# interestingLSY/swiftLLM

Measured on AMD Instinct MI355X. Metric: decode tok/s (llama3-8b bfloat16, batch 32/GPU, 1024-in/128-out; prefill tok/s alongside), higher is better.
Workload: dtype bf16

## Files before the change

include/swiftllm_hip.h:

```cpp
#ifndef SWIFTLLM_HIP_H
#define SWIFTLLM_HIP_H

#include <stddef.h>
#include <stdint.h>

#ifdef __cplusplus
extern "C" {
#endif

#define SWL_ABI_VERSION 2

#define SWL_F16 0
#define SWL_BF16 1

#define SWL_OK 0
#define SWL_ERR_BAD_ARG (-1)
#define SWL_ERR_UNSUPPORTED (-2)
#define SWL_ERR_LAUNCH (-3)
#define SWL_ERR_RUNTIME (-4)

typedef void *swl_stream_t;

int swl_abi_version(void);
const char *swl_strerror(int code);
// ... 215 lines not shown
int swl_gemm_packed_wide_silu_gate(void *out, const void *x, const void *w_up_gate_packed, int32_t M, int32_t I,
                                   int32_t K, int64_t x_row_stride, int64_t out_row_stride, int32_t waves_per_group,
                                   int32_t dtype, swl_stream_t stream);
int swl_gemm_packed_mid_partial(float *slabs, size_t slabs_bytes, const void *x, const void *w_packed, int32_t M,
                                int32_t N, int32_t K, int64_t x_row_stride, int32_t k_splits, int32_t dtype,
                                swl_stream_t stream);

int swl_gemm_skinny_choose_splits(int32_t N, int32_t K);
int swl_gemm_skinny_packed_choose_splits(int32_t N, int32_t K);
int swl_gemm_skinny_partial(float *slabs, size_t slabs_bytes, const void *x, const void *w, int32_t M,
                            int32_t N, int32_t K, int64_t x_row_stride, int32_t k_splits,
                            int32_t dtype, swl_stream_t stream);
int swl_splitk_reduce(void *out, const float *slabs, int32_t k_splits, int32_t M, int32_t N,
                      int64_t out_row_stride, int32_t dtype, swl_stream_t stream);
int swl_splitk_fused_add_rmsnorm(void *x_out, void *residual, const void *w, float eps,
                                 const float *slabs, int32_t k_splits, int64_t num_tokens,
                                 int32_t hidden, int32_t dtype, swl_stream_t stream);
int swl_splitk_rotary_store_kv_decode(void *q_out, void *k_out, void *v_out, const float *qkv_slabs,
                                      int32_t k_splits, const void *cos_table, const void *sin_table,
                                      const int32_t *pos_idx, void *k_cache, void *v_cache,
                                      const int32_t *block_table, const int32_t *seq_ids,
                                      const int32_t *seq_lens, int32_t num_decoding_seqs,
                                      int32_t num_q_heads, int32_t num_kv_heads, int32_t head_dim,
                                      int32_t cur_layer, int32_t num_layers, int32_t block_size,
                                      int32_t max_blocks_per_seq, int64_t q_tok_stride,
                                      int64_t k_tok_stride, int64_t v_tok_stride, int32_t dtype,
                                      swl_stream_t stream);

int swl_decode_positions(int32_t *pos_idx, const int32_t *seq_lens, int32_t num_decoding_seqs,
                         swl_stream_t stream);

int swl_splitk_add_scale(void *x_scaled, void *residual, const void *w, const float *slabs, int32_t k_splits,
                         float *ssq_out, int64_t num_tokens, int32_t hidden, int32_t dtype, swl_stream_t stream);
int swl_gemm_skinny_packed_silu_gate_rs(void *out, const void *x, const void *w_up_gate_packed, const float *row_ssq,
                                        int32_t ssq_parts, float eps, int32_t M, int32_t I, int32_t K,
                                        int64_t x_row_stride, int64_t out_row_stride, int32_t dtype, swl_stream_t stream);
int swl_paged_attn_decode_qkv_rs(void *o, const float *qkv_slabs, int32_t k_splits, const float *row_ssq,
                                 int32_t ssq_parts, int32_t hidden, float eps, const void *cos_table,
                                 const void *sin_table, const int32_t *pos_idx, void *k_cache, void *v_cache,
                                 const int32_t *block_table, const int32_t *seq_ids, const int32_t *seq_lens,
                                 void *scratch, float softmax_scale, int32_t num_decoding_seqs, int32_t num_q_heads,
                                 int32_t num_kv_heads, int32_t head_dim, int32_t num_layers, int32_t block_size,
                                 int32_t cur_layer, int32_t max_blocks_per_seq, int32_t seq_block_size,
                                 int32_t num_seq_blocks, int64_t o_tok_stride, int32_t dtype, swl_stream_t stream);

int swl_paged_attn_decode_qkv_rs_partials(void *o, const float *qkv_slabs, int32_t k_splits, const float *row_ssq,
                                          int32_t ssq_parts, int32_t hidden, float eps, const void *cos_table,
                                          const void *sin_table, const int32_t *pos_idx, void *k_cache, void *v_cache,
                                          const int32_t *block_table, const int32_t *seq_ids, const int32_t *seq_lens,
                                          void *scratch, float softmax_scale, int32_t num_decoding_seqs,
                                          int32_t num_q_heads, int32_t num_kv_heads, int32_t head_dim,
                                          int32_t num_layers, int32_t block_size, int32_t cur_layer,
                                          int32_t max_blocks_per_seq, int32_t seq_block_size, int32_t num_seq_blocks,
                                          int64_t o_tok_stride, int32_t dtype, swl_stream_t stream);
int swl_gemm_tiny_partial_from_attn(float *slabs_out, size_t slabs_out_bytes, int32_t k_splits_out,
                                    const float *attn_scratch, const int32_t *seq_lens, int32_t num_q_heads,
                                    int32_t head_dim, int32_t seq_block_size, int32_t num_seq_blocks,
                                    const void *w_packed, int32_t M, int32_t N, int32_t dtype, swl_stream_t stream);
int swl_gemm_tiny_max_tokens(void);
int swl_gemm_tiny_partial_from_splitk(float *slabs_out, size_t slabs_out_bytes, int32_t k_splits_out, float *ssq_out,
                                      const float *slabs_in, int32_t k_splits_in, const void *residual_in,
                                      void *residual_out, const void *norm_w, const void *w_packed, int32_t M, int32_t N,
                                      int32_t K, int32_t dtype, swl_stream_t stream);
int swl_gemm_tiny_silu_gate_from_splitk(void *out, const float *slabs_in, int32_t k_splits_in, const void *residual_in,
                                        void *residual_out, const void *norm_w, float eps, const void *w_up_gate_packed,
                                        int32_t M, int32_t I, int32_t K, int64_t out_row_stride, int32_t dtype,
// ... 49 lines not shown
```

swiftllm_amd/_hip.py:

```python
import ctypes
import os
import threading

import torch

_LIB_NAME = "libswiftllm_hip.so"
_LIB_PATH = os.path.join(os.path.dirname(os.path.abspath(__file__)), "csrc", _LIB_NAME)

SWL_F16 = 0
SWL_BF16 = 1
ABI_VERSION = 2

_P = ctypes.c_void_p
_I32 = ctypes.c_int32
_I64 = ctypes.c_int64
_F32 = ctypes.c_float

SIGNATURES = {
    "swl_rmsnorm": [_P, _P, _F32, _I64, _I32, _I32, _P],
    "swl_fused_add_rmsnorm": [_P, _P, _P, _F32, _I64, _I32, _I32, _P],
    "swl_rotary": [_P, _P, _P, _P, _P, _I64, _I32, _I32, _I32, _I64, _I64, _I32, _P],
    "swl_store_kv_prefill": [_P, _P, _P, _P, _P, _P, _P, _P, _I32, _I32, _I32, _I32, _I32, _I32,
                             _I32, _I32, _I64, _I64, _I32, _P],
    "swl_store_kv_decode": [_P, _P, _P, _P, _P, _P, _P, _I32, _I32, _I32, _I32, _I32, _I32, _I32,
# ... 49 lines not shown
    "swl_gemm_skinny_partial": [_P, ctypes.c_size_t, _P, _P, _I32, _I32, _I32, _I64, _I32, _I32, _P],
    "swl_splitk_reduce": [_P, _P, _I32, _I32, _I32, _I64, _I32, _P],
    "swl_gemm_skinny_silu_gate": [_P, _P, _P, _I32, _I32, _I32, _I64, _I64, _I32, _P],
    "swl_splitk_fused_add_rmsnorm": [_P, _P, _P, _F32, _P, _I32, _I64, _I32, _I32, _P],
    "swl_splitk_add_scale": [_P, _P, _P, _P, _I32, _P, _I64, _I32, _I32, _P],
    "swl_gemm_skinny_packed_silu_gate_rs": [_P, _P, _P, _P, _I32, _F32, _I32, _I32, _I32, _I64, _I64, _I32, _P],
    "swl_paged_attn_decode_qkv_rs": [_P, _P, _I32, _P, _I32, _I32, _F32, _P, _P, _P, _P, _P, _P, _P, _P, _P, _F32, _I32,
                                     _I32, _I32, _I32, _I32, _I32, _I32, _I32, _I32, _I32, _I64, _I32, _P],
    "swl_splitk_rotary_store_kv_decode": [_P, _P, _P, _P, _I32, _P, _P, _P, _P, _P, _P, _P, _P, _I32, _I32,
                                          _I32, _I32, _I32, _I32, _I32, _I32, _I64, _I64, _I64, _I32, _P],
    "swl_paged_attn_decode_qkv_rs_partials": [_P, _P, _I32, _P, _I32, _I32, _F32, _P, _P, _P, _P, _P, _P, _P, _P, _P, _F32,
                                              _I32, _I32, _I32, _I32, _I32, _I32, _I32, _I32, _I32, _I32, _I64, _I32, _P],
    "swl_gemm_tiny_partial_from_attn": [_P, ctypes.c_size_t, _I32, _P, _P, _I32, _I32, _I32, _I32, _P, _I32, _I32, _I32, _P],
    "swl_gemm_tiny_partial_from_splitk": [_P, ctypes.c_size_t, _I32, _P, _P, _I32, _P, _P, _P, _P, _I32, _I32, _I32, _I32, _P],
    "swl_gemm_tiny_silu_gate_from_splitk": [_P, _P, _I32, _P, _P, _P, _F32, _P, _I32, _I32, _I32, _I64, _I32, _P],
    "swl_gemm_rows_add": [_P, _P, _P, _I32, _I32, _I32, _I64, _I32, _P],
    "swl_gemm_skinny_packed_partial_nf": [_P, ctypes.c_size_t, _P, _P, _P, _P, _I32, _I32, _I32, _I64, _I32, _I32, _P],
    "swl_gemm_skinny_packed_silu_gate_nf": [_P, _P, _P, _F32, _P, _I32, _I32, _I32, _I64, _I64, _I32, _P],
    "swl_gemm_rows_add_ssq": [_P, _P, _P, _P, _I32, _I32, _I32, _I64, _I32, _P],
    "swl_gemm_skinny_packed_silu_gate_nx": [_P, _P, _P, _F32, _P, _I32, _P, _I32, _I32, _I32, _I64, _I64, _I32, _P],
    "swl_gemm_skinny_packed_partial_nx": [_P, ctypes.c_size_t, _P, _P, _F32, _P, _I32, _P, _I32, _I32, _I32, _I64, _I32, _I32, _P],
    "swl_decode_engine_reset": [_P, ctypes.c_size_t, _P],
    "swl_decode_engine_step": [_P, _P, _P, _P, _P, _P, _P, _P, _P, _P, _P, _P, _P, ctypes.c_size_t, _P, _P, _I32, _I32,
                               _I32, _I32, _I32, _I32, _I32, _F32, _F32, _I32, _I32, _P],
}
_SPECIAL = {
    "swl_abi_version": ([], _I32),
    "swl_strerror": ([_I32], ctypes.c_char_p),
    "swl_paged_attn_scratch_bytes": ([_I32, _I32, _I32, _I32], ctypes.c_size_t),
    "swl_argmax_scratch_bytes": ([_I64], ctypes.c_size_t),
    "swl_gemm_skinny_workspace_bytes": ([_I32, _I32, _I32], ctypes.c_size_t),
    "swl_gemm_skinny_choose_splits": ([_I32, _I32], _I32),
    "swl_gemm_skinny_packed_choose_splits": ([_I32, _I32], _I32),
    "swl_gemm_packed_mid_choose_splits": ([_I32, _I32, _I32], _I32),
    "swl_gemm_packed_wide_workspace_bytes": ([_I32, _I32, _I32], ctypes.c_size_t),
    "swl_gemm_packed_wide_choose_splits": ([_I32, _I32, _I32], _I32),
    "swl_gemm_tiny_max_tokens": ([], _I32),
    "swl_gemm_rows_supported": ([_I32, _I32, _I32], _I32),
    "swl_decode_engine_supported": ([_I32, _I32, _I32, _I32, _I32, _I32], _I32),
    "swl_decode_engine_slots_per_layer": ([_I32, _I32, _I32, _I32], _I32),
    "swl_decode_engine_workspace_bytes": ([_I32, _I32, _I32, _I32], ctypes.c_size_t),
    "swl_paged_attn_verify_max_tokens": ([_I32, _I32], _I32),
    "swl_paged_attn_verify": ([_P, _P, _P, _P, _P, _P, _P, _P, _P, _P, _F32, _I32, _I32, _I32, _I32, _I32, _I32, _I32,
                               _I32, _I32, _I32, _I32, _I32, _I32, _I64, _I64, _I32, _P], _I32),
    "swl_logits_adjust": ([_P, _I64, _I32, _I64, _I32, _P, _P, _P, _P, _P, _P], _I32),
    "swl_lora_k_splits": ([_I32], _I32),
    "swl_lora_shrink": ([_P, _P, _P, _P, _P, _I32, _I32, _I32, _I32, _I32, _I64, _I32, _P], _I32),
    "swl_lora_expand": ([_P, _P, _P, _P, _P, _P, _P, _I32, _I32, _I32, _I32, _I32, _I32, _I32, _I32, _I64, _I32, _P], _I32),
}

_lock = threading.Lock()
_lib = None


class HipLibraryError(RuntimeError):
    """libswiftllm_hip.so is missing, stale, or a kernel entry point returned an error code."""


def library_path() -> str:
    return os.environ.get("SWIFTLLM_HIP_LIB", _LIB_PATH)


def load():
    global _lib
    if _lib is not None:
        return _lib
# ... 71 lines not shown
```

swiftllm_amd/csrc/build.py:

```python
import argparse
import concurrent.futures
import os
import shutil
import subprocess
import tempfile

HERE = os.path.dirname(os.path.abspath(__file__))
ROOT = os.path.dirname(os.path.dirname(HERE))
SOURCES = [
    "rmsnorm.hip",
    "rotary.hip",
    "kvcache.hip",
    "silu_mul.hip",
    "paged_attn.hip",
    "paged_attn_verify.hip",
    "prefill_attn.hip",
    "prefill_attn_paged.hip",
    "kvcache_fp8.hip",
    "paged_attn_fp8.hip",
    "block_table.hip",
    "swap_blocks.hip",
    "gemm_skinny.hip",
    "gemm_tiny.hip",
    "gemm_wide.hip",
    "gemm_rows.hip",
    "argmax.hip",
    "sampling.hip",
    "logits_adjust.hip",
    "lora.hip",
    "decode_engine.hip",
]
HEADERS = ["swl_common.h", "attend_block.h", "attn_mfma.h", "decode_attn.h", "prefill_tile.h", "fp8_kv.h", "gemm_host.h", os.path.join(ROOT, "include", "swiftllm_hip.h")]
LIB = os.path.join(HERE, "libswiftllm_hip.so")
OBJ_DIR = os.path.join(HERE, "build")
ARCH = "gfx950"
CXXFLAGS = [f"--offload-arch={ARCH}", "-O3", "-std=c++17", "-fPIC", "-ffp-contract=off", "-Wall",
            "-Wno-unused-function"]


def _hipcc() -> str:
    for cand in (os.environ.get("HIPCC"), shutil.which("hipcc"), "/opt/rocm/bin/hipcc"):
        if cand and os.path.exists(cand):
            return cand
    raise RuntimeError("hipcc not found (set HIPCC or install ROCm under /opt/rocm)")


def _newer(target: str, deps) -> bool:
    if not os.path.exists(target):
        return False
    t = os.path.getmtime(target)
    return all(os.path.getmtime(d) <= t for d in deps)


def build(force: bool = False, jobs: int = 0, verbose: bool = True, tag: str = "", defines=(), swap=None) -> str:
    hipcc = _hipcc()
    obj_dir = os.path.join(tempfile.gettempdir(), "swiftllm_hip_variants", tag) if tag else OBJ_DIR
    lib = os.path.join(HERE, f"libswiftllm_hip_{tag}.so") if tag else LIB
    return _build(hipcc, obj_dir, lib, [f"-D{d}" for d in defines], force, jobs, verbose, swap or {})


def _build(hipcc, OBJ_DIR, LIB, extra, force, jobs, verbose, swap) -> str:
    os.makedirs(OBJ_DIR, exist_ok=True)
    hdrs = [h if os.path.isabs(h) else os.path.join(HERE, h) for h in HEADERS]
    hdrs.append(os.path.abspath(__file__))
    todo, objs = [], []
# ... 41 lines not shown
```

swiftllm_amd/csrc/gemm_skinny.hip:

```cpp
#include "gemm_host.h"

namespace swl {

__device__ __forceinline__ float16_t mfma32x32x16(vec8_t<f16> a, vec8_t<f16> b, float16_t c) {
    return __builtin_amdgcn_mfma_f32_32x32x16_f16(a, b, c, 0, 0, 0);
}
__device__ __forceinline__ float16_t mfma32x32x16(vec8_t<bf16> a, vec8_t<bf16> b, float16_t c) {
    return __builtin_amdgcn_mfma_f32_32x32x16_bf16(a, b, c, 0, 0, 0);
}

constexpr int kKT = 128;
constexpr int kGemmWaves = 4;

enum GemmMode {
    kGemmDirect = 0,
    kGemmPartial = 1,
    kGemmSiluGate = 2,
};

struct GemmExtra {
    int k_tiles_total;
    const float *ssq_in;
    float eps;
    int ssq_parts;
    const void *norm_w;
    float *ssq_out;
};

template <typename T, int MODE>
__device__ __forceinline__ void gemm_epilogue(const float16_t &acc, void *__restrict__ out_, T *wtiles,
                                              int wave_pitch, int wave, int lane, bool is_gate, bool tile_ok,
                                              int col0, int n0, int ksplit, int M, int N, int64_t out_stride,
                                              float rs = 1.0f, int gate_waves_off = 2) {
    const int l32 = lane & 31;
    const int hf = lane >> 5;
    if constexpr (MODE == kGemmSiluGate) {
        T *mine = wtiles + wave * wave_pitch;
        if (is_gate) {
#pragma unroll
            for (int r = 0; r < 16; ++r) {
                const float g = to_f(to_t<T>(acc[r] * rs));
                mine[l32 * 40 + (r & 3) + 8 * (r >> 2) + 4 * hf] = to_t<T>(g / (1.0f + expf(-g)));
            }
        }
        __syncthreads();
// ... 337 lines not shown
        }
        gemm_epilogue<T, MODE>(acc, out_, &lds[0][0], 32 * 40, wave, lane, is_gate, tile_ok, col0, n0, ksplit, M, N,
                               out_stride, rs, HWV);
    } else {
        gemm_epilogue<T, MODE>(acc, out_, &lds[PACKED ? 0 : 2][0], 32 * kKT, wave, lane, is_gate, tile_ok, col0, n0,
                               ksplit, M, N, out_stride);
    }
}

template <typename T>
__global__ __launch_bounds__(256) void splitk_reduce_kernel(T *__restrict__ out,
                                                            const float *__restrict__ slabs, int M,
                                                            int N, int KS, int64_t out_stride) {
    const int n4 = N >> 2;
    const int64_t items = static_cast<int64_t>(M) * n4;
    for (int64_t it = blockIdx.x * 256ll + threadIdx.x; it < items;
         it += static_cast<int64_t>(gridDim.x) * 256ll) {
        const int m = static_cast<int>(it / n4);
        const int c = static_cast<int>(it - static_cast<int64_t>(m) * n4);
        float4_t s = {0.f, 0.f, 0.f, 0.f};
        for (int k = 0; k < KS; ++k) {
            const float4_t v = *reinterpret_cast<const float4_t *>(
                slabs + (static_cast<int64_t>(k) * M + m) * N + 4 * c);
            s += v;
        }
        typedef T vec4 __attribute__((ext_vector_type(4)));
        vec4 o;
#pragma unroll
        for (int e = 0; e < 4; ++e) o[e] = to_t<T>(s[e]);
        *reinterpret_cast<vec4 *>(out + static_cast<int64_t>(m) * out_stride + 4 * c) = o;
    }
}

static int choose_k_splits(int N, int K) {
    const int tiles = N / 32;
    int ks = 1;
    while (ks < 16 && tiles * ks < 768 && K % (kKT * ks * 2) == 0 && K / (ks * 2) >= 2 * kKT) ks *= 2;
    return ks;
}

static int choose_k_splits_packed(int N, int K, bool *uneven) {
    const int even = choose_k_splits(N, K);
    *uneven = false;
    const int tiles = N / 32, ktiles = K / kKT;
    if (tiles * even >= 512) return even;
    int ks = even;
    while (ks < 16 && tiles * ks < 768 && ktiles / (ks * 2) >= 8) ks *= 2;
    if (ks == even) return even;
    *uneven = K % (kKT * ks) != 0;
    return ks;
}

static bool use_ring(int kc) { return kc / kKT >= 8; }

template <typename T>
void launch_splitk_reduce(T *out, const float *slabs, int ks, int M, int N, int64_t out_row_stride, hipStream_t stream) {
    const int64_t items = static_cast<int64_t>(M) * (N / 4);
    hipLaunchKernelGGL((splitk_reduce_kernel<T>), dim3(static_cast<unsigned>((items + 255) / 256)), dim3(256), 0, stream,
                       out, slabs, M, N, ks, out_row_stride);
}
template void launch_splitk_reduce<f16>(f16 *, const float *, int, int, int, int64_t, hipStream_t);
template void launch_splitk_reduce<bf16>(bf16 *, const float *, int, int, int, int64_t, hipStream_t);

template <int MODE>
static int four_wave_groups(int N) {
    return MODE == kGemmSiluGate ? (N / 32 + 1) / 2 : (N / 32 + kGemmWaves - 1) / kGemmWaves;
}

static GemmArgs silu_gate_args(void *out, const void *x, const void *w, int M, int I, int K, int64_t x_row_stride,
                               int64_t out_row_stride, int max_m = 32) {
    return GemmArgs{out, x, w, nullptr, 0, M, I, K, x_row_stride, out_row_stride, 1, max_m, kKT};
}

template <typename T, int MODE>
static void launch_rowmajor(const GemmArgs &a, hipStream_t stream, void *dst, int64_t dst_stride, int kc, int ks) {
    const dim3 grid(four_wave_groups<MODE>(a.N), ks);
    const T *x = static_cast<const T *>(a.x), *w = static_cast<const T *>(a.w);
    if (use_ring(kc))
        hipLaunchKernelGGL((gemm_skinny_ring_kernel<T, MODE>), grid, dim3(kGemmWaves * 64), 0, stream, dst, x, w, a.M, a.N,
                           a.K, kc, a.x_row_stride, dst_stride, GemmExtra{});
    else
        hipLaunchKernelGGL((gemm_skinny_kernel<T, MODE>), grid, dim3(kGemmWaves * 64), 0, stream, dst, x, w, a.M, a.N, a.K,
                           kc, a.x_row_stride, dst_stride);
}

template <typename T>
static int run_gemm(const GemmArgs &a, hipStream_t stream) {
    const int ks = a.k_splits > 0 ? a.k_splits : choose_k_splits(a.N, a.K);
    if (a.K % (kKT * ks) != 0) return SWL_ERR_UNSUPPORTED;
    const int kc = a.K / ks;
    return run_splitk<T>(
        a, ks, stream,
        [&](void *out) { launch_rowmajor<T, kGemmDirect>(a, stream, out, a.out_row_stride, kc, ks); },
        [&](float *slabs) { launch_rowmajor<T, kGemmPartial>(a, stream, slabs, a.N, kc, ks); });
}

}

extern "C" size_t swl_gemm_skinny_workspace_bytes(int32_t M, int32_t N, int32_t K) {
// ... 40 lines not shown
    if (!out || !slabs || out_row_stride < N || (out_row_stride & 3)) return SWL_ERR_BAD_ARG;
    if (!swl::aligned16(slabs) || (reinterpret_cast<uintptr_t>(out) & 7u)) return SWL_ERR_BAD_ARG;
    SWL_DISPATCH_DTYPE(dtype, T, {
        swl::launch_splitk_reduce<T>(static_cast<T *>(out), slabs, k_splits, M, N, out_row_stride,
                                     static_cast<hipStream_t>(stream));
    });
    return swl::check_launch();
}

extern "C" int swl_gemm_skinny_silu_gate(void *out, const void *x, const void *w_up_gate, int32_t M,
                                         int32_t I, int32_t K, int64_t x_row_stride,
                                         int64_t out_row_stride, int32_t dtype, swl_stream_t stream) {
    const swl::GemmArgs a = swl::silu_gate_args(out, x, w_up_gate, M, I, K, x_row_stride, out_row_stride);
    int rc;
    if (swl::gemm_args_settled(a, rc)) return rc;
    SWL_DISPATCH_DTYPE(dtype, T, {
        swl::launch_rowmajor<T, swl::kGemmSiluGate>(a, static_cast<hipStream_t>(stream), out, out_row_stride, K, 1);
    });
    return swl::check_launch();
}

namespace swl {

template <typename T>
__global__ __launch_bounds__(256) void pack_weight_kernel(T *__restrict__ dst, const T *__restrict__ src, int N, int K) {
    const int64_t blocks = static_cast<int64_t>(N / 32) * (K / 16);
    const int lane = threadIdx.x & 63;
    for (int64_t b = blockIdx.x * 4ll + (threadIdx.x >> 6); b < blocks; b += gridDim.x * 4ll) {
        const int64_t nt = b / (K / 16);
        const int k16 = static_cast<int>(b - nt * (K / 16));
        const T *s = src + (nt * 32 + (lane & 31)) * K + k16 * 16 + 8 * (lane >> 5);
        store8(dst + (b * 64 + lane) * 8, load8(s));
    }
}

static bool prefer_three_waves(int N, int ks) {
    const int tiles = N / 32;
    if (tiles % 3 != 0) return false;
    const int wg4 = (tiles + kGemmWaves - 1) / kGemmWaves * ks, wg3 = tiles / 3 * ks;
    return wg4 < 256 && wg3 <= 256;
}

static bool silu_gate_two_waves(int M) {
    static const int forced = [] { const char *e = getenv("SWL_SILU_WAVES"); return !e ? 0 : e[0] == '2' ? 2 : e[0] == '4' ? 4 : 0; }();
    return forced ? forced == 2 : M <= 8;
}

template <typename T, int MODE, bool NF = false, bool NX = false>
static void launch_packed_ring(const GemmArgs &a, hipStream_t stream, void *dst, int64_t dst_stride, int kc, int ks,
                               const GemmExtra &fuse = GemmExtra{}) {
    const int tiles = a.N / 32;
    auto launch = [&](auto rd, auto nwv, int groups) {
        constexpr int RD = decltype(rd)::value, NWV = decltype(nwv)::value;
        hipLaunchKernelGGL((gemm_skinny_ring_kernel<T, MODE, true, RD, NWV, NF, NX>), dim3(groups, ks), dim3(NWV * 64), 0,
                           stream, dst, static_cast<const T *>(a.x), static_cast<const T *>(a.w), a.M, a.N, a.K, kc,
                           a.x_row_stride, dst_stride, fuse);
    };
    const bool deep = use_ring(kc);
    if constexpr (MODE == kGemmPartial) {
        if (fuse.k_tiles_total == 0 && prefer_three_waves(a.N, ks)) {
            if (NF || !deep) return launch(IntTag<2>{}, IntTag<3>{}, tiles / 3);
            if constexpr (!NF) return launch(IntTag<3>{}, IntTag<3>{}, tiles / 3);
        }
    }
    if constexpr (MODE == kGemmSiluGate && NF) {
        if (deep && (NX ? a.M <= 8 : silu_gate_two_waves(a.M))) return launch(IntTag<3>{}, IntTag<2>{}, tiles);
    }
    const int groups = four_wave_groups<MODE>(a.N);
    if (deep) return launch(IntTag<3>{}, IntTag<kGemmWaves>{}, groups);
    if constexpr (!(MODE == kGemmSiluGate && NX)) launch(IntTag<2>{}, IntTag<kGemmWaves>{}, groups);
}

template <typename T>
static int run_gemm_packed(const GemmArgs &a, hipStream_t stream) {
    bool uneven = false;
    int ks = a.k_splits;
    if (ks <= 0) ks = choose_k_splits_packed(a.N, a.K, &uneven);
    else uneven = a.K % (kKT * ks) != 0;
    if (uneven && (a.K / kKT) / ks < 8) return SWL_ERR_UNSUPPORTED;
    const int kc = uneven ? (a.K / kKT / ks) * kKT : a.K / ks;
    GemmExtra fuse{};
    fuse.k_tiles_total = uneven ? a.K / kKT : 0;
    return run_splitk<T>(
        a, ks, stream, [&](void *out) { launch_packed_ring<T, kGemmDirect>(a, stream, out, a.out_row_stride, kc, ks); },
        [&](float *slabs) { launch_packed_ring<T, kGemmPartial>(a, stream, slabs, a.N, kc, ks, fuse); });
}

}

extern "C" int swl_gemm_pack_weight(void *dst, const void *src, int32_t N, int32_t K, int32_t dtype,
                                    swl_stream_t stream) {
    if (N <= 0 || K <= 0 || !dst || !src || dst == src) return SWL_ERR_BAD_ARG;
    if ((N & 31) || (K & 15)) return SWL_ERR_UNSUPPORTED;
    if (!swl::aligned16(dst) || !swl::aligned16(src)) return SWL_ERR_BAD_ARG;
    const int64_t blocks = static_cast<int64_t>(N / 32) * (K / 16);
    const unsigned grid = static_cast<unsigned>(blocks / 4 + 1 < 65536 ? blocks / 4 + 1 : 65536);
    SWL_DISPATCH_DTYPE(dtype, T, {
        hipLaunchKernelGGL((swl::pack_weight_kernel<T>), dim3(grid), dim3(256), 0, static_cast<hipStream_t>(stream),
                           static_cast<T *>(dst), static_cast<const T *>(src), N, K);
    });
    return swl::check_launch();
}

extern "C" int swl_gemm_skinny_packed(void *out, const void *x, const void *w_packed, void *workspace,
                                      size_t workspace_bytes, int32_t M, int32_t N, int32_t K, int64_t x_row_stride,
                                      int64_t out_row_stride, int32_t k_splits, int32_t dtype, swl_stream_t stream) {
    const swl::GemmArgs a{out, x, w_packed, workspace, workspace_bytes, M, N, K, x_row_stride, out_row_stride, k_splits, 32,
                          swl::kKT};
    int rc;
    if (swl::gemm_args_settled(a, rc)) return rc;
    SWL_DISPATCH_DTYPE(dtype, T, { return swl::run_gemm_packed<T>(a, static_cast<hipStream_t>(stream)); });
}

extern "C" int swl_gemm_skinny_packed_partial(float *slabs, size_t slabs_bytes, const void *x, const void *w_packed,
                                              int32_t M, int32_t N, int32_t K, int64_t x_row_stride,
// ... 370 lines not shown
```

swiftllm_amd/csrc/rmsnorm.hip:

```cpp
#include "swl_common.h"

namespace swl {

template <int NWAVES>
__device__ __forceinline__ float block_allreduce_sum(float v, float *lds) {
    v = wave_allreduce_sum(v);
    if constexpr (NWAVES > 1) {
        const int wave = threadIdx.x >> 6;
        if ((threadIdx.x & 63) == 0) lds[wave] = v;
        __syncthreads();
        float t = 0.f;
#pragma unroll
        for (int i = 0; i < NWAVES; ++i) t += lds[i];
        v = t;
    }
    return v;
}

template <typename T, int NT, int VPT, bool FUSED_ADD>
__global__ __launch_bounds__(NT) void rmsnorm_kernel(T *__restrict__ x, T *__restrict__ residual,
                                                     const T *__restrict__ w, float eps, int hidden,
                                                     const float *__restrict__ slabs, int ks,
                                                     int64_t slab_stride) {
    __shared__ float red[NT / 64];
    const int64_t row = blockIdx.x;
    const int nvec = hidden >> 3;
    T *xr = x + row * hidden;
    T *rr = FUSED_ADD ? residual + row * hidden : nullptr;

    vec8_t<T> wv[VPT];
#pragma unroll
    for (int i = 0; i < VPT; ++i) {
        const int v = threadIdx.x + i * NT;
// ... 11 lines not shown
                vec8_t<T> rv = load8(rr + v * 8);
#pragma unroll
                for (int j = 0; j < 8; ++j) xv[j] = add_t<T>(xv[j], rv[j]);
                store8(rr + v * 8, xv);
            }
#pragma unroll
            for (int j = 0; j < 8; ++j) {
                vals[i][j] = to_f(xv[j]);
                ssq = fmaf(vals[i][j], vals[i][j], ssq);
            }
        } else {
#pragma unroll
            for (int j = 0; j < 8; ++j) vals[i][j] = 0.f;
        }
    }
    ssq = block_allreduce_sum<NT / 64>(ssq, red);
    const float variance = ssq / static_cast<float>(hidden);
    const float rstd = 1.0f / sqrtf(variance + eps);
#pragma unroll
    for (int i = 0; i < VPT; ++i) {
        const int v = threadIdx.x + i * NT;
        if (v < nvec) {
            vec8_t<T> ov;
#pragma unroll
            for (int j = 0; j < 8; ++j) ov[j] = to_t<T>(vals[i][j] * rstd * to_f(wv[i][j]));
            store8(xr + v * 8, ov);
        }
    }
}

constexpr int kAddScaleThreads = 128;
constexpr int kAddScaleChunk = kAddScaleThreads * 8;

template <typename T>
__global__ __launch_bounds__(kAddScaleThreads) void splitk_add_scale_kernel(
    T *__restrict__ xs, T *__restrict__ residual, const T *__restrict__ w, const float *__restrict__ slabs, int ks,
    int64_t slab_stride, float *__restrict__ ssq_out, int num_tokens, int hidden) {
    __shared__ float red[kAddScaleThreads / 64];
    const int part = blockIdx.x, row = blockIdx.y;
    const int col = part * kAddScaleChunk + threadIdx.x * 8;
    const int64_t off = static_cast<int64_t>(row) * hidden + col;
    const vec8_t<T> wv = load8(w + col);
    const vec8_t<T> rv = load8(residual + off);
    vec8_t<T> xv = load8_splitk<T>(slabs, ks, slab_stride, off);
    vec8_t<T> sv;
    float ssq = 0.f;
#pragma unroll
    for (int j = 0; j < 8; ++j) {
        xv[j] = add_t<T>(xv[j], rv[j]);
        const float v = to_f(xv[j]);
        ssq = fmaf(v, v, ssq);
        sv[j] = to_t<T>(v * to_f(wv[j]));
    }
    store8(residual + off, xv);
    store8(xs + off, sv);
    ssq = block_allreduce_sum<kAddScaleThreads / 64>(ssq, red);
    if (threadIdx.x == 0) ssq_out[static_cast<int64_t>(part) * num_tokens + row] = ssq;
}

template <typename T, bool FUSED_ADD>
static int launch_rmsnorm(T *x, T *residual, const T *w, float eps, int64_t num_tokens, int hidden,
                          hipStream_t stream, const float *slabs = nullptr, int ks = 0) {
    const int64_t slab_stride = num_tokens * hidden;
    const int nvec = hidden / 8;
    const dim3 grid(static_cast<unsigned>(num_tokens));
#define SWL_RMS_CASE(NT, VPT)                                                                    \
    hipLaunchKernelGGL((rmsnorm_kernel<T, NT, VPT, FUSED_ADD>), grid, dim3(NT), 0, stream, x,    \
                       residual, w, eps, hidden, slabs, ks, slab_stride)
    if (nvec <= 64) SWL_RMS_CASE(64, 1);
    else if (nvec <= 128) SWL_RMS_CASE(128, 1);
    else if (nvec <= 256) SWL_RMS_CASE(256, 1);
// ... 33 lines not shown
        return swl::launch_rmsnorm<T, true>(static_cast<T *>(x), static_cast<T *>(residual),
                                            static_cast<const T *>(w), eps, num_tokens, hidden,
                                            static_cast<hipStream_t>(stream));
    });
}

extern "C" int swl_splitk_fused_add_rmsnorm(void *x_out, void *residual, const void *w, float eps,
                                            const float *slabs, int32_t k_splits,
                                            int64_t num_tokens, int32_t hidden, int32_t dtype,
                                            swl_stream_t stream) {
    if (num_tokens < 0 || hidden <= 0 || (hidden & 7) || k_splits <= 0) return SWL_ERR_BAD_ARG;
    if (num_tokens == 0) return SWL_OK;
    if (!x_out || !residual || !w || !slabs || !swl::aligned16(x_out) || !swl::aligned16(residual) ||
        !swl::aligned16(w) || !swl::aligned16(slabs))
        return SWL_ERR_BAD_ARG;
    if (num_tokens > 0x7fffffffLL) return SWL_ERR_UNSUPPORTED;
    SWL_DISPATCH_DTYPE(dtype, T, {
        return swl::launch_rmsnorm<T, true>(static_cast<T *>(x_out), static_cast<T *>(residual),
                                            static_cast<const T *>(w), eps, num_tokens, hidden,
                                            static_cast<hipStream_t>(stream), slabs, k_splits);
    });
}

extern "C" int swl_splitk_add_scale(void *x_scaled, void *residual, const void *w, const float *slabs, int32_t k_splits,
                                    float *ssq_out, int64_t num_tokens, int32_t hidden, int32_t dtype,
                                    swl_stream_t stream) {
    if (num_tokens < 0 || hidden <= 0 || k_splits <= 0) return SWL_ERR_BAD_ARG;
    if (num_tokens == 0) return SWL_OK;
    if (hidden % swl::kAddScaleChunk) return SWL_ERR_UNSUPPORTED;
    if (!x_scaled || !residual || !w || !slabs || !ssq_out || !swl::aligned16(x_scaled) || !swl::aligned16(residual) ||
        !swl::aligned16(w) || !swl::aligned16(slabs))
        return SWL_ERR_BAD_ARG;
    if (num_tokens > 65535) return SWL_ERR_UNSUPPORTED;
    const dim3 grid(hidden / swl::kAddScaleChunk, static_cast<unsigned>(num_tokens));
    SWL_DISPATCH_DTYPE(dtype, T, {
        hipLaunchKernelGGL((swl::splitk_add_scale_kernel<T>), grid, dim3(swl::kAddScaleThreads), 0,
                           static_cast<hipStream_t>(stream), static_cast<T *>(x_scaled), static_cast<T *>(residual),
                           static_cast<const T *>(w), slabs, k_splits, num_tokens * static_cast<int64_t>(hidden), ssq_out,
                           static_cast<int>(num_tokens), hidden);
    });
    return swl::check_launch();
}
```

swiftllm_amd/engine_config.py:

```python
import argparse
import dataclasses


@dataclasses.dataclass
class EngineConfig:
    model_path: str
    use_dummy: bool

    block_size: int
    gpu_mem_utilization: float
    num_cpu_blocks: int
    max_seqs_in_block_table: int
    max_blocks_per_seq: int

    max_batch_size: int
    max_tokens_in_batch: int

    dtype: str = "float16"
    fuse_qkv: bool = True
    use_hip_graph: bool = True
    use_skinny_gemm: bool = True
    pack_decode_weights: bool = True
    tuning: dict = None
    max_prefill_chunk: int = 0
    kv_cache_dtype: str = "auto"
    speculative_ngram: int = 0
    speculative_max_batch: int = 8
    max_loras: int = 0
    max_lora_rank: int = 16
    lora_modules: list = None

    TUNING_DEFAULTS = dict(
        fuse_rope_kvstore=True,
        fuse_splitk_consumers=True,
        fuse_rope_into_attention=True,
        defer_rmsnorm=True,
        tiny_decode_batches=True,
        rows_decode=True,
        decode_engine=False,
        pin_swap_memory=True,
        pause_gc_while_serving=True,
    )

    SUPPORTED_BLOCK_SIZE = 16
    KV_CACHE_DTYPES = ("auto", "fp8_e4m3")
    LORA_RANKS = (8, 16, 32, 64)

    def __post_init__(self):
        if int(self.block_size) != self.SUPPORTED_BLOCK_SIZE:
            raise ValueError(
                f"block_size={self.block_size} is not supported: the MI355X kernels are built for "
                f"{self.SUPPORTED_BLOCK_SIZE}-token KV blocks (pass --block-size {self.SUPPORTED_BLOCK_SIZE})")
        if self.dtype not in ("float16", "bfloat16"):
            raise ValueError(f"dtype must be 'float16' or 'bfloat16', got {self.dtype!r}")
        if int(self.max_prefill_chunk) < 0:
            raise ValueError(f"max_prefill_chunk must be >= 0 (0 = off), got {self.max_prefill_chunk}")
        if self.kv_cache_dtype not in self.KV_CACHE_DTYPES:
            raise ValueError(f"kv_cache_dtype must be one of {list(self.KV_CACHE_DTYPES)}, got {self.kv_cache_dtype!r}")
        if int(self.speculative_ngram) < 0:
            raise ValueError(f"speculative_ngram must be >= 0 (0 = off), got {self.speculative_ngram}")
        if int(self.speculative_max_batch) < 0:
            raise ValueError(f"speculative_max_batch must be >= 0, got {self.speculative_max_batch}")
        if int(self.max_loras) < 0:
            raise ValueError(f"max_loras must be >= 0 (0 = off), got {self.max_loras}")
        if int(self.max_lora_rank) not in self.LORA_RANKS:
            raise ValueError(f"max_lora_rank must be one of {list(self.LORA_RANKS)}, got {self.max_lora_rank}")
        if self.lora_modules:
            if int(self.max_loras) <= 0:
                raise ValueError("lora_modules needs max_loras > 0")
            names = [str(m).partition("=")[0] for m in self.lora_modules]
            if any("=" not in str(m) or not n or not str(m).partition("=")[2] for m, n in zip(self.lora_modules, names)):
                raise ValueError(f"lora_modules entries are 'NAME=PATH' strings, got {list(self.lora_modules)}")
# ... 66 lines not shown
```

swiftllm_amd/worker/model.py:

```python
import math
import os
import time
from typing import List, Optional

import torch

from swiftllm_amd import _hip
from swiftllm_amd.engine_config import EngineConfig
from swiftllm_amd.model_config import LlamaModelConfig
from swiftllm_amd.sampling_params import SamplingParams, is_greedy
from swiftllm_amd.utils import GB

from .batch_plan import BatchPlan, plan_batch, plan_verify
from .block_manager import BlockManager
from . import decode_engine as _decode_engine
from .infer_state import LlamaInferState
from .kernels.block_swapping import swap_blocks
from .kernels.linear import RawResidual
from .kernels.paged_attn import verify_max_tokens
from .kernels.rmsnorm import fused_add_rmsnorm_from_splitk, rmsnorm_inplace
from .kernels import logits_process
from .kernels.sampling import device_args, pack_params
from .lora import LoraBatch, LoraStaging, LoraStep, LoraStore, parse_lora_modules, rows_of_sequences
from .layers.pre_layer import LlamaPreLayer
from .layers.transformer_layer import LlamaTransformerLayer
from .layers.post_layer import LlamaPostLayer
from .token_history import TokenHistory, row_entries
from .weight import load_weights, pack_decode_weights

_DTYPES = {"float16": torch.float16, "fp16": torch.float16, "half": torch.float16,
           "bfloat16": torch.bfloat16, "bf16": torch.bfloat16}


def _require_hip_device():
    if not torch.cuda.is_available():
        raise _hip.HipLibraryError(
            "no HIP device visible: swiftllm_amd's data plane runs only on an AMD GPU (gfx950) "
            "through libswiftllm_hip.so; there is no CPU path")
    _hip.load()


class _DecodeGraph:
    __slots__ = ("graph", "out_tokens", "logits", "seq_block_size", "num_seq_blocks", "engine")


class _DecodeLookahead:
    __slots__ = ("seq_ids", "lens", "tokens", "plan", "dev", "sampling", "processed")


class LlamaModel:

    @torch.inference_mode()
    def __init__(self, engine_config: EngineConfig):
        self.engine_config = engine_config
        self.model_config = LlamaModelConfig.load_from_model_path(engine_config.model_path)
        self.dtype = _DTYPES[getattr(engine_config, "dtype", "float16")]
        self.device = torch.device("cuda")
        self.kv_fp8 = getattr(engine_config, "kv_cache_dtype", "auto") == "fp8_e4m3"
        self.kv_dtype = torch.float8_e4m3fn if self.kv_fp8 else self.dtype
        self.kv_scales = self.kv_inv_scales = None

        self.weight = None
        self._cos_cached = self._sin_cached = None
        self.pre_layer = None
# ... 79 lines not shown
    @torch.inference_mode()
    def unload_lora(self, name: str) -> int:
        return self._require_lora_store().unload(name)

    def loras(self) -> dict:
        return {} if self.lora_store is None else self.lora_store.names()

    def _tune_routes(self):
        ecfg = self.engine_config
        if not (getattr(ecfg, "use_skinny_gemm", False) and getattr(ecfg, "pack_decode_weights", False)
                and ecfg.max_batch_size > 64):
            return
        from .kernels.linear import tune_wide_routes
        stats = tune_wide_routes(self.weight.projection_tensors(), [lw.up_gate_proj for lw in self.weight.layers[:1]],
                                 self.dtype, self.device, ecfg.model_path)
        if stats.get("measured") or stats.get("read"):
            print(f"[Model] decode-projection routing: {stats['measured']} (shape, bucket) classes measured, "
                  f"{stats['read']} read from {stats['path']}", flush=True)

    @torch.inference_mode()
    def repack_decode_weights(self):
        ecfg = self.engine_config
        if getattr(ecfg, "pack_decode_weights", False) and getattr(ecfg, "use_skinny_gemm", False):
            proj_bytes = sum(t.numel() * t.element_size() for t in self.weight.projection_tensors())
            free_b, total_b = torch.cuda.mem_get_info(self.device)
            usable = total_b * float(getattr(ecfg, "gpu_mem_utilization", 0.97)) - (total_b - free_b)
            if proj_bytes > 0.75 * usable:
                print(f"[Model] pack_decode_weights disabled: a second {proj_bytes / 2**30:.1f} GiB copy of the "
                      f"projection weights would leave {max(0.0, usable - proj_bytes) / 2**30:.1f} GiB for the KV "
                      f"pool; decode GEMMs stream the row-major weights instead", flush=True)
                ecfg.pack_decode_weights = False
                return
            pack_decode_weights(self.weight)
        for layer in self.transformer_layers or ():
            layer.refresh_facts()
        self._build_decode_engine()

    def _build_decode_engine(self):
        ecfg, cfg = self.engine_config, self.model_config
        self._engine = None
        if not (getattr(ecfg, "decode_engine", False) and getattr(ecfg, "use_skinny_gemm", False)):
            return
        num_cus = torch.cuda.get_device_properties(self.device).multi_processor_count
        if cfg.head_dim != 128 or not _decode_engine.supported(cfg, num_cus):
            return
        need = _decode_engine.stream_bytes(cfg, torch.empty((), dtype=self.dtype).element_size())
        free_b, total_b = torch.cuda.mem_get_info(self.device)
        usable = total_b * float(getattr(ecfg, "gpu_mem_utilization", 0.97)) - (total_b - free_b)
        if need > 0.75 * usable:
            print(f"[Model] decode_engine disabled: its {need / 2**30:.1f} GiB weight stream would leave "
                  f"{max(0.0, usable - need) / 2**30:.1f} GiB for the KV pool", flush=True)
            return
        self._engine = _decode_engine.DecodeEngine(cfg, self.weight, self.dtype, self.device)

    @torch.inference_mode()
    def profile_num_blocks(self) -> int:
        ecfg = self.engine_config
        torch.cuda.empty_cache()
        torch.cuda.reset_peak_memory_stats()
        num_tokens, batch = ecfg.max_tokens_in_batch, ecfg.max_batch_size
        lens = [num_tokens // batch] * batch
        lens[-1] += num_tokens % batch
        self.k_cache = self.v_cache = None
        self.forward([[0] * n for n in lens], list(range(batch)), [], ignore_kvcache=True)
        torch.cuda.synchronize()
        free_memory, total_memory = torch.cuda.mem_get_info()
        peak_memory = total_memory - free_memory
        usable = total_memory * ecfg.gpu_mem_utilization
        print(f"[Model.profile] GPU total memory: {total_memory / GB:.2f} GB, "
# ... 715 lines not shown
```

Measured before the change: 7633.

## Prefetch next layer's packed QKV weights into cache during add-scale kernel

```diff
diff --git a/include/swiftllm_hip.h b/include/swiftllm_hip.h
--- a/include/swiftllm_hip.h
+++ b/include/swiftllm_hip.h
@@ -271,6 +271,10 @@
 
 int swl_splitk_add_scale(void *x_scaled, void *residual, const void *w, const float *slabs, int32_t k_splits,
                          float *ssq_out, int64_t num_tokens, int32_t hidden, int32_t dtype, swl_stream_t stream);
+int swl_weight_chain_set(const void *key, const void *w_packed, int32_t N, int32_t K, int32_t dtype);
+int swl_weight_chain_clear(void);
+int swl_weight_chain_plan(const void *key, int32_t num_tokens, int32_t hidden, int64_t *out, int32_t cap);
+
 int swl_gemm_skinny_packed_silu_gate_rs(void *out, const void *x, const void *w_up_gate_packed, const float *row_ssq,
                                         int32_t ssq_parts, float eps, int32_t M, int32_t I, int32_t K,
                                         int64_t x_row_stride, int64_t out_row_stride, int32_t dtype, swl_stream_t stream);
diff --git a/swiftllm_amd/_hip.py b/swiftllm_amd/_hip.py
--- a/swiftllm_amd/_hip.py
+++ b/swiftllm_amd/_hip.py
@@ -105,6 +105,9 @@
     "swl_gemm_skinny_workspace_bytes": ([_I32, _I32, _I32], ctypes.c_size_t),
     "swl_gemm_skinny_choose_splits": ([_I32, _I32], _I32),
     "swl_gemm_skinny_packed_choose_splits": ([_I32, _I32], _I32),
+    "swl_weight_chain_set": ([_P, _P, _I32, _I32, _I32], _I32),
+    "swl_weight_chain_clear": ([], _I32),
+    "swl_weight_chain_plan": ([_P, _I32, _I32, _P, _I32], _I32),
     "swl_gemm_packed_mid_choose_splits": ([_I32, _I32, _I32], _I32),
     "swl_gemm_packed_wide_workspace_bytes": ([_I32, _I32, _I32], ctypes.c_size_t),
     "swl_gemm_packed_wide_choose_splits": ([_I32, _I32, _I32], _I32),
diff --git a/swiftllm_amd/csrc/build.py b/swiftllm_amd/csrc/build.py
--- a/swiftllm_amd/csrc/build.py
+++ b/swiftllm_amd/csrc/build.py
@@ -21,6 +21,7 @@
     "block_table.hip",
     "swap_blocks.hip",
     "gemm_skinny.hip",
+    "weight_chain.hip",
     "gemm_tiny.hip",
     "gemm_wide.hip",
     "gemm_rows.hip",
@@ -30,7 +31,7 @@
     "lora.hip",
     "decode_engine.hip",
 ]
-HEADERS = ["swl_common.h", "attend_block.h", "attn_mfma.h", "decode_attn.h", "prefill_tile.h", "fp8_kv.h", "gemm_host.h", os.path.join(ROOT, "include", "swiftllm_hip.h")]
+HEADERS = ["swl_common.h", "attend_block.h", "attn_mfma.h", "decode_attn.h", "prefill_tile.h", "fp8_kv.h", "gemm_host.h", "weight_chain.h", os.path.join(ROOT, "include", "swiftllm_hip.h")]
 LIB = os.path.join(HERE, "libswiftllm_hip.so")
 OBJ_DIR = os.path.join(HERE, "build")
 ARCH = "gfx950"
diff --git a/swiftllm_amd/csrc/gemm_skinny.hip b/swiftllm_amd/csrc/gemm_skinny.hip
--- a/swiftllm_amd/csrc/gemm_skinny.hip
+++ b/swiftllm_amd/csrc/gemm_skinny.hip
@@ -1,4 +1,5 @@
 #include "gemm_host.h"
+#include "weight_chain.h"
 
 namespace swl {
 
@@ -8,9 +9,6 @@
 __device__ __forceinline__ float16_t mfma32x32x16(vec8_t<bf16> a, vec8_t<bf16> b, float16_t c) {
     return __builtin_amdgcn_mfma_f32_32x32x16_bf16(a, b, c, 0, 0, 0);
 }
-
-constexpr int kKT = 128;
-constexpr int kGemmWaves = 4;
 
 enum GemmMode {
     kGemmDirect = 0,
@@ -414,26 +412,6 @@
     }
 }
 
-static int choose_k_splits(int N, int K) {
-    const int tiles = N / 32;
-    int ks = 1;
-    while (ks < 16 && tiles * ks < 768 && K % (kKT * ks * 2) == 0 && K / (ks * 2) >= 2 * kKT) ks *= 2;
-    return ks;
-}
-
-static int choose_k_splits_packed(int N, int K, bool *uneven) {
-    const int even = choose_k_splits(N, K);
-    *uneven = false;
-    const int tiles = N / 32, ktiles = K / kKT;
-    if (tiles * even >= 512) return even;
-    int ks = even;
-    while (ks < 16 && tiles * ks < 768 && ktiles / (ks * 2) >= 8) ks *= 2;
-    if (ks == even) return even;
-    *uneven = K % (kKT * ks) != 0;
-    return ks;
-}
-
-static bool use_ring(int kc) { return kc / kKT >= 8; }
 
 template <typename T>
 void launch_splitk_reduce(T *out, const float *slabs, int ks, int M, int N, int64_t out_row_stride, hipStream_t stream) {
@@ -446,7 +424,7 @@
 
 template <int MODE>
 static int four_wave_groups(int N) {
-    return MODE == kGemmSiluGate ? (N / 32 + 1) / 2 : (N / 32 + kGemmWaves - 1) / kGemmWaves;
+    return MODE == kGemmSiluGate ? (N / 32 + 1) / 2 : partial_groups(N, kGemmWaves);
 }
 
 static GemmArgs silu_gate_args(void *out, const void *x, const void *w, int M, int I, int K, int64_t x_row_stride,
@@ -553,13 +531,6 @@
         const T *s = src + (nt * 32 + (lane & 31)) * K + k16 * 16 + 8 * (lane >> 5);
         store8(dst + (b * 64 + lane) * 8, load8(s));
     }
-}
-
-static bool prefer_three_waves(int N, int ks) {
-    const int tiles = N / 32;
-    if (tiles % 3 != 0) return false;
-    const int wg4 = (tiles + kGemmWaves - 1) / kGemmWaves * ks, wg3 = tiles / 3 * ks;
-    return wg4 < 256 && wg3 <= 256;
 }
 
 static bool silu_gate_two_waves(int M) {
@@ -579,9 +550,9 @@
     };
     const bool deep = use_ring(kc);
     if constexpr (MODE == kGemmPartial) {
-        if (fuse.k_tiles_total == 0 && prefer_three_waves(a.N, ks)) {
-            if (NF || !deep) return launch(IntTag<2>{}, IntTag<3>{}, tiles / 3);
-            if constexpr (!NF) return launch(IntTag<3>{}, IntTag<3>{}, tiles / 3);
+        if (partial_waves(a.N, ks, fuse.k_tiles_total != 0) == 3) {
+            if (NF || !deep) return launch(IntTag<2>{}, IntTag<3>{}, partial_groups(a.N, 3));
+            if constexpr (!NF) return launch(IntTag<3>{}, IntTag<3>{}, partial_groups(a.N, 3));
         }
     }
     if constexpr (MODE == kGemmSiluGate && NF) {
@@ -594,14 +565,11 @@
 
 template <typename T>
 static int run_gemm_packed(const GemmArgs &a, hipStream_t stream) {
-    bool uneven = false;
-    int ks = a.k_splits;
-    if (ks <= 0) ks = choose_k_splits_packed(a.N, a.K, &uneven);
-    else uneven = a.K % (kKT * ks) != 0;
-    if (uneven && (a.K / kKT) / ks < 8) return SWL_ERR_UNSUPPORTED;
-    const int kc = uneven ? (a.K / kKT / ks) * kKT : a.K / ks;
+    PackedSplit s;
+    if (!packed_split(a.N, a.K, a.k_splits, s)) return SWL_ERR_UNSUPPORTED;
+    const int ks = s.ks, kc = s.kc;
     GemmExtra fuse{};
-    fuse.k_tiles_total = uneven ? a.K / kKT : 0;
+    fuse.k_tiles_total = s.uneven ? a.K / kKT : 0;
     return run_splitk<T>(
         a, ks, stream, [&](void *out) { launch_packed_ring<T, kGemmDirect>(a, stream, out, a.out_row_stride, kc, ks); },
         [&](float *slabs) { launch_packed_ring<T, kGemmPartial>(a, stream, slabs, a.N, kc, ks, fuse); });
diff --git a/swiftllm_amd/csrc/rmsnorm.hip b/swiftllm_amd/csrc/rmsnorm.hip
--- a/swiftllm_amd/csrc/rmsnorm.hip
+++ b/swiftllm_amd/csrc/rmsnorm.hip
@@ -1,4 +1,5 @@
 #include "swl_common.h"
+#include "weight_chain.h"
 
 namespace swl {
 
@@ -76,11 +77,36 @@
 constexpr int kAddScaleThreads = 128;
 constexpr int kAddScaleChunk = kAddScaleThreads * 8;
 
+static_assert(kWarmThreads == kAddScaleThreads, "the warming workgroups are workgroups of this launch");
+
+__device__ __forceinline__ void warm_next_weights(const WarmPlan &p, int e) {
+    if (e >= p.extra) return;
+    const int lane = threadIdx.x & 63;
+    const WarmShare s(p, e, __builtin_amdgcn_readfirstlane(threadIdx.x >> 6));
+    typedef unsigned int u4 __attribute__((ext_vector_type(4)));
+    const char *base = p.w + lane * 128;
+    for (int q = s.u; q < s.Q; q += s.U) {
+        const WarmGroup g(p, s.c + 8 * q);
+        const char *src = base + g.base;
+        u4 v[kGemmWaves * kWarmTilesMax];
+#pragma unroll
+        for (int i = 0; i < kGemmWaves * kWarmTilesMax; ++i) {
+            const int wv = i / kWarmTilesMax, t = i % kWarmTilesMax;
+            v[i] = u4{0, 0, 0, 0};
+            if (wv < g.n_waves && t < g.n_tiles) v[i] = *reinterpret_cast<const u4 *>(src + wv * g.wave_pitch + t * p.tile_bytes);
+        }
+#pragma unroll
+        for (int i = 0; i < kGemmWaves * kWarmTilesMax; ++i) asm volatile("" ::"v"(v[i]));
+    }
+}
+
 template <typename T>
 __global__ __launch_bounds__(kAddScaleThreads) void splitk_add_scale_kernel(
     T *__restrict__ xs, T *__restrict__ residual, const T *__restrict__ w, const float *__restrict__ slabs, int ks,
-    int64_t slab_stride, float *__restrict__ ssq_out, int num_tokens, int hidden) {
+    int64_t slab_stride, float *__restrict__ ssq_out, int num_tokens, int hidden, WarmPlan warm) {
     __shared__ float red[kAddScaleThreads / 64];
+    if (static_cast<int>(blockIdx.y) >= num_tokens)
+        return warm_next_weights(warm, (static_cast<int>(blockIdx.y) - num_tokens) * gridDim.x + blockIdx.x);
     const int part = blockIdx.x, row = blockIdx.y;
     const int col = part * kAddScaleChunk + threadIdx.x * 8;
     const int64_t off = static_cast<int64_t>(row) * hidden + col;
@@ -180,12 +206,16 @@
         !swl::aligned16(w) || !swl::aligned16(slabs))
         return SWL_ERR_BAD_ARG;
     if (num_tokens > 65535) return SWL_ERR_UNSUPPORTED;
-    const dim3 grid(hidden / swl::kAddScaleChunk, static_cast<unsigned>(num_tokens));
+    const int parts = hidden / swl::kAddScaleChunk;
+    swl::WarmPlan warm;
+    const int warm_rows = swl::warm_plan_for(w, num_tokens, parts * static_cast<int>(num_tokens), warm)
+                              ? (warm.extra + parts - 1) / parts : 0;
+    const dim3 grid(parts, static_cast<unsigned>(num_tokens) + warm_rows);
     SWL_DISPATCH_DTYPE(dtype, T, {
         hipLaunchKernelGGL((swl::splitk_add_scale_kernel<T>), grid, dim3(swl::kAddScaleThreads), 0,
                            static_cast<hipStream_t>(stream), static_cast<T *>(x_scaled), static_cast<T *>(residual),
                            static_cast<const T *>(w), slabs, k_splits, num_tokens * static_cast<int64_t>(hidden), ssq_out,
-                           static_cast<int>(num_tokens), hidden);
+                           static_cast<int>(num_tokens), hidden, warm);
     });
     return swl::check_launch();
 }
diff --git a/swiftllm_amd/csrc/weight_chain.h b/swiftllm_amd/csrc/weight_chain.h
--- /dev/null
+++ b/swiftllm_amd/csrc/weight_chain.h
@@ -0,0 +1,104 @@
+#pragma once
+
+#include "swl_common.h"
+
+namespace swl {
+
+constexpr int kKT = 128;
+constexpr int kGemmWaves = 4;
+
+static int choose_k_splits(int N, int K) {
+    const int tiles = N / 32;
+    int ks = 1;
+    while (ks < 16 && tiles * ks < 768 && K % (kKT * ks * 2) == 0 && K / (ks * 2) >= 2 * kKT) ks *= 2;
+    return ks;
+}
+
+static int choose_k_splits_packed(int N, int K, bool *uneven) {
+    const int even = choose_k_splits(N, K);
+    *uneven = false;
+    const int tiles = N / 32, ktiles = K / kKT;
+    if (tiles * even >= 512) return even;
+    int ks = even;
+    while (ks < 16 && tiles * ks < 768 && ktiles / (ks * 2) >= 8) ks *= 2;
+    if (ks == even) return even;
+    *uneven = K % (kKT * ks) != 0;
+    return ks;
+}
+
+static bool use_ring(int kc) { return kc / kKT >= 8; }
+
+static bool prefer_three_waves(int N, int ks) {
+    const int tiles = N / 32;
+    if (tiles % 3 != 0) return false;
+    const int wg4 = (tiles + kGemmWaves - 1) / kGemmWaves * ks, wg3 = tiles / 3 * ks;
+    return wg4 < 256 && wg3 <= 256;
+}
+
+struct PackedSplit {
+    int ks;
+    bool uneven;
+    int kc;
+};
+
+inline bool packed_split(int N, int K, int k_splits, PackedSplit &s) {
+    s.uneven = false;
+    s.ks = k_splits;
+    if (s.ks <= 0) s.ks = choose_k_splits_packed(N, K, &s.uneven);
+    else s.uneven = K % (kKT * s.ks) != 0;
+    if (s.uneven && (K / kKT) / s.ks < 8) return false;
+    s.kc = s.uneven ? (K / kKT / s.ks) * kKT : K / s.ks;
+    return true;
+}
+
+inline int partial_waves(int N, int ks, bool uneven) { return !uneven && prefer_three_waves(N, ks) ? 3 : kGemmWaves; }
+inline int partial_groups(int N, int waves) { return (N / 32 + waves - 1) / waves; }
+
+constexpr int kWarmMaxTokens = 32;
+constexpr int kWarmThreads = 128;
+constexpr int kWarmMaxGroups = 256;
+constexpr int kWarmTilesDefault = 1;
+constexpr int kWarmTilesMax = 4;
+
+struct WarmPlan {
+    const char *w;
+    int groups;
+    int lks;
+    int waves;
+    int tiles;
+    int k_tiles;
+    int depth;
+    int tile_bytes;
+    int first;
+    int extra;
+};
+
+struct WarmShare {
+    int c, u, U, Q;
+    __host__ __device__ WarmShare(const WarmPlan &p, int e, int wave) {
+        constexpr int kWavesPerGroup = kWarmThreads / 64;
+        c = (p.first + e) & 7;
+        u = (e >> 3) * kWavesPerGroup + wave;
+        U = (p.extra >> 3) * kWavesPerGroup;
+        const int wgs = p.groups << p.lks;
+        Q = wgs > c ? (wgs - c + 7) >> 3 : 0;
+    }
+};
+
+struct WarmGroup {
+    int64_t base, wave_pitch;
+    int n_waves, n_tiles;
+    __host__ __device__ WarmGroup(const WarmPlan &p, int j) {
+        const int by = j / p.groups, bx = j - by * p.groups;
+        const int t0 = (by * p.k_tiles) >> p.lks, t1 = ((by + 1) * p.k_tiles) >> p.lks;
+        const int left = p.tiles - bx * p.waves;
+        n_waves = left < p.waves ? left : p.waves;
+        n_tiles = t1 - t0 < p.depth ? t1 - t0 : p.depth;
+        wave_pitch = static_cast<int64_t>(p.k_tiles) * p.tile_bytes;
+        base = static_cast<int64_t>(bx * p.waves) * wave_pitch + static_cast<int64_t>(t0) * p.tile_bytes;
+    }
+};
+
+bool warm_plan_for(const void *key, int64_t num_tokens, int consumer_groups, WarmPlan &p);
+
+}
diff --git a/swiftllm_amd/csrc/weight_chain.hip b/swiftllm_amd/csrc/weight_chain.hip
--- /dev/null
+++ b/swiftllm_amd/csrc/weight_chain.hip
@@ -0,0 +1,103 @@
+#include "weight_chain.h"
+
+#include <cstdlib>
+#include <mutex>
+#include <unordered_map>
+
+namespace swl {
+namespace {
+
+struct ChainEntry {
+    const void *w_packed;
+    int N, K, dtype;
+};
+
+std::mutex g_chain_mutex;
+std::unordered_map<const void *, ChainEntry> g_chain;
+
+int warm_depth() {
+    static const int depth = [] {
+        const char *e = getenv("SWL_WARM_TILES");
+        return e && e[0] >= '0' && e[0] <= '0' + kWarmTilesMax && !e[1] ? e[0] - '0' : kWarmTilesDefault;
+    }();
+    return depth;
+}
+
+}
+
+bool warm_plan_for(const void *key, int64_t num_tokens, int consumer_groups, WarmPlan &p) {
+    p = WarmPlan{};
+    if (num_tokens <= 0 || num_tokens > kWarmMaxTokens || consumer_groups <= 0 || warm_depth() == 0) return false;
+    ChainEntry e;
+    {
+        std::lock_guard<std::mutex> lock(g_chain_mutex);
+        const auto it = g_chain.find(key);
+        if (it == g_chain.end()) return false;
+        e = it->second;
+    }
+    PackedSplit s;
+    if (!packed_split(e.N, e.K, 0, s)) return false;
+    int lks = 0;
+    while ((1 << lks) < s.ks) ++lks;
+    p.waves = partial_waves(e.N, s.ks, s.uneven);
+    p.groups = partial_groups(e.N, p.waves);
+    p.lks = lks;
+    p.tiles = e.N / 32;
+    p.k_tiles = e.K / kKT;
+    p.depth = warm_depth();
+    p.tile_bytes = 32 * kKT * 2;
+    p.first = consumer_groups;
+    const int per_xcd = ((p.groups << lks) + 7) / 8;
+    const int groups_per_xcd = (per_xcd + kWarmThreads / 64 - 1) / (kWarmThreads / 64);
+    p.extra = 8 * groups_per_xcd < kWarmMaxGroups ? 8 * groups_per_xcd : kWarmMaxGroups;
+    const int64_t extent = static_cast<int64_t>(e.N) * e.K * 2;
+    if ((1 << lks) != s.ks || static_cast<int64_t>(p.tiles) * p.k_tiles * p.tile_bytes > extent) return false;
+    p.w = static_cast<const char *>(e.w_packed);
+    return true;
+}
+
+}
+
+extern "C" int swl_weight_chain_set(const void *key, const void *w_packed, int32_t N, int32_t K, int32_t dtype) {
+    if (!key || !w_packed || N <= 0 || K <= 0 || !swl::aligned16(w_packed)) return SWL_ERR_BAD_ARG;
+    if (dtype != SWL_F16 && dtype != SWL_BF16) return SWL_ERR_BAD_ARG;
+    if ((N & 31) || (K & (swl::kKT - 1))) return SWL_ERR_UNSUPPORTED;
+    swl::PackedSplit s;
+    if (!swl::packed_split(N, K, 0, s)) return SWL_ERR_UNSUPPORTED;
+    std::lock_guard<std::mutex> lock(swl::g_chain_mutex);
+    swl::g_chain[key] = swl::ChainEntry{w_packed, N, K, dtype};
+    return SWL_OK;
+}
+
+extern "C" int swl_weight_chain_clear(void) {
+    std::lock_guard<std::mutex> lock(swl::g_chain_mutex);
+    swl::g_chain.clear();
+    return SWL_OK;
+}
+
+extern "C" int swl_weight_chain_plan(const void *key, int32_t num_tokens, int32_t hidden, int64_t *out, int32_t cap) {
+    swl::WarmPlan p;
+    if (!out || hidden <= 0 || hidden % 1024 || !swl::warm_plan_for(key, num_tokens, hidden / 1024 * num_tokens, p)) return 0;
+    int n = 8, units = 0;
+    for (int e = 0; e < p.extra; ++e)
+        for (int wave = 0; wave < swl::kWarmThreads / 64; ++wave) {
+            const swl::WarmShare s(p, e, wave);
+            for (int q = s.u; q < s.Q; q += s.U) {
+                const int j = s.c + 8 * q;
+                const swl::WarmGroup g(p, j);
+                for (int w = 0; w < g.n_waves; ++w)
+                    for (int t = 0; t < g.n_tiles; ++t) {
+                        if (n + 5 <= cap) {
+                            const int64_t row[5] = {e, j, w, t, g.base + w * g.wave_pitch + static_cast<int64_t>(t) * p.tile_bytes};
+                            for (int i = 0; i < 5; ++i) out[n + i] = row[i];
+                        }
+                        n += 5;
+                        ++units;
+                    }
+            }
+        }
+    if (n > cap) return -n;
+    const int64_t head[8] = {p.groups, 1 << p.lks, p.waves, p.depth, p.extra, p.tile_bytes, p.first, units};
+    for (int i = 0; i < 8; ++i) out[i] = head[i];
+    return n;
+}
diff --git a/swiftllm_amd/engine_config.py b/swiftllm_amd/engine_config.py
--- a/swiftllm_amd/engine_config.py
+++ b/swiftllm_amd/engine_config.py
@@ -38,6 +38,7 @@
         tiny_decode_batches=True,
         rows_decode=True,
         decode_engine=False,
+        warm_next_weights=True,
         pin_swap_memory=True,
         pause_gc_while_serving=True,
     )
diff --git a/swiftllm_amd/worker/model.py b/swiftllm_amd/worker/model.py
--- a/swiftllm_amd/worker/model.py
+++ b/swiftllm_amd/worker/model.py
@@ -1,6 +1,7 @@
 import math
 import os
 import time
+import weakref
 from typing import List, Optional
 
 import torch
@@ -30,6 +31,9 @@
 
 _DTYPES = {"float16": torch.float16, "fp16": torch.float16, "half": torch.float16,
            "bfloat16": torch.bfloat16, "bf16": torch.bfloat16}
+
+
+_weight_chain_owner = None
 
 
 def _require_hip_device():
@@ -175,9 +179,38 @@
                 ecfg.pack_decode_weights = False
                 return
             pack_decode_weights(self.weight)
+        self._register_weight_chain()
         for layer in self.transformer_layers or ():
             layer.refresh_facts()
         self._build_decode_engine()
+
+    def _register_weight_chain(self):
+        global _weight_chain_owner
+        lib = _hip.load()
+        lib.swl_weight_chain_clear()
+        _weight_chain_owner = weakref.ref(self)
+        self._drop_decode_graphs()
+        self._lookahead = None
+        if not getattr(self.engine_config, "warm_next_weights", False) or self.weight is None:
+            return
+        for lw in self.weight.layers:
+            packed = getattr(lw.qkv_proj, "_swl_packed", None) if lw.qkv_proj is not None else None
+            if packed is None:
+                continue
+            n, k = lw.qkv_proj.shape
+            lib.swl_weight_chain_set(_hip.ptr(lw.attn_norm), _hip.ptr(packed), n, k, _hip.dtype_code(packed.dtype))
+
+    def close(self):
+        global _weight_chain_owner
+        if _weight_chain_owner is not None and _weight_chain_owner() in (self, None):
+            _weight_chain_owner = None
+            try:
+                _hip.load().swl_weight_chain_clear()
+            except Exception:
+                pass
+
+    def __del__(self):
+        self.close()
 
     def _build_decode_engine(self):
         ecfg, cfg = self.engine_config, self.model_config
```

Result: no change. 7650, median of 2 (+0.2%).
